# AlexanderKazakov/gcm

Hardware: AMD Instinct MI355X
Metric: Mnode-steps/sec + achieved HBM GB/s, 3D isotropic elastic 512³ CubicGrid (higher is better)
Workload: dtype f64; 1 GPU; 3-D isotropic elastic CubicGrid 512^3, borderSize 2, Courant 0.9, tau 0.9, one full time step (3 stages); global_nodes=134217728, slabs=1, launch=single process, parallelism=single, fp=fma

## Files before the change

gcm_amd/csrc/gcmx.hip:

```cpp
#include <rccl/rccl.h>

#include <algorithm>
#include <chrono>
#include <cmath>
#include <condition_variable>
#include <cstdio>
#include <cstdlib>
#include <cstring>
#include <memory>
#include <mutex>
#include <string>
#include <thread>
#include <vector>

#include "../../include/gcmx.h"
#include "common.hpp"
#include "launch.hpp"
#include "ortho.hpp"

using namespace gcmx;
static_assert(GCMX_MAX_BORDER_Q == kMaxBorderQ, "border quantity limit");
static_assert(GCMX_MAX_FACE_CONDITIONS == kMaxFaceConds && GCMX_NO_FACE_CONDITION == kNoFaceCond, "face maps");

namespace {
// ... 193 lines not shown
		if (!c->prof) return;
		b = bucket_id(c, name);
		a = take_event(c);
		e = take_event(c);
		(void)hipEventRecord(a, st);
	}
	~Timed() {
		if (b < 0) return;
		(void)hipEventRecord(e, st);
		c->pending.push_back({b, bytes, a, e});
		if (kname) c->buckets[b].kernel = kname;
	}
};

void drain_timings(gcmx_ctx* c) {
	for (auto& p : c->pending) {
		float ms = 0;
		(void)hipEventSynchronize(p.b);
		(void)hipEventElapsedTime(&ms, p.a, p.b);
		c->buckets[p.bucket].total_ms += ms;
		c->buckets[p.bucket].launches += 1;
		c->buckets[p.bucket].bytes += p.bytes;
		c->event_pool.push_back(p.a);
		c->event_pool.push_back(p.b);
	}
	c->pending.clear();
}

long long round_up(long long v, long long m) { return (v + m - 1) / m * m; }

static long long layout_pad(const char* name, long long align) {
	const char* e = std::getenv(name);
	const long long v = (e && *e) ? std::atoll(e) : 0;
	return v > 0 ? round_up(v, align) : 0;
}

long long dev_offset(const Geo& g, const int it[3]) {
	long long o = g.origin;
	for (int d = 0; d < g.D; d++) o += (long long)it[d] * g.stride[d];
	return o;
}

gcmx_status check_ctx(gcmx_ctx* c) {
	if (!c) return fail(GCMX_ERR_INVALID_ARG, "null context");
	if (hipSetDevice(c->device) != hipSuccess) return fail(GCMX_ERR_HIP, "hipSetDevice failed");
	return GCMX_OK;
}

gcmx_status build_tables(gcmx_ctx* c, double tau) {
	if (c->n_mat <= 0) return fail(GCMX_ERR_STATE, "materials not set");
	if (std::memcmp(&tau, &c->tabs_tau, sizeof(double)) == 0) return GCMX_OK;
	const int D = c->D, M = c->M, bs = c->bs;
	std::vector<AxisTable> h((size_t)c->n_mat * D);
	for (int m = 0; m < c->n_mat; m++)
		for (int s = 0; s < D; s++) {
			AxisTable& t = h[(size_t)m * D + s];
			std::memset(&t, 0, sizeof(t));
			const double* Um = &c->U[((size_t)m * D + s) * M * M];
			const double* U1m = &c->U1[((size_t)m * D + s) * M * M];
			const double* Lm = &c->L[((size_t)m * D + s) * M];
			for (int i = 0; i < M * M; i++) {
				t.U[i] = Um[i];
				t.U1[i] = U1m[i];
			}
			for (int k = 0; k < M; k++) {
				const double dx = Lm[k] * (-tau);
				const double q = std::fabs(dx) / c->desc.h[s];
// ... 2297 lines not shown
```

gcm_amd/csrc/iso.hpp:

```cpp
#pragma once

#include "common.hpp"
#include "launch.hpp"

namespace gcmx {


__host__ __device__ constexpr int sig3(int i, int j) {
	return (i <= j) ? 3 + (i * 3 - ((i - 1) * i) / 2 + j - i)
	                : 3 + (j * 3 - ((j - 1) * j) / 2 + i - j);
}
__host__ __device__ constexpr unsigned bit(int i) { return 1u << i; }

__host__ __device__ constexpr int tang1(int s) { return s == 0 ? 1 : 0; }
__host__ __device__ constexpr int tang2(int s) { return s == 2 ? 1 : 2; }
__host__ __device__ constexpr int sgn1(int s) { return s == 0 ? -1 : 1; }
__host__ __device__ constexpr int sgn2(int s) { return s == 2 ? 1 : -1; }

enum Slot : int { kZero = 0, kOne, kHalf, kA, kB, kG, kP1, kP2, kS };
struct Coef {
	int slot;
	int sign;
};
__host__ __device__ constexpr Coef cz() { return Coef{kZero, 0}; }
// ... 190 lines not shown
		for (int j = 0; j < kMaxM; j++) b[j] = sgpr_ptr(p + j * cs);
	}
	__device__ __forceinline__ void st(int j, unsigned off, double v) const {
		typedef __attribute__((address_space(1))) char* gb;
		*reinterpret_cast<gptr>(reinterpret_cast<gb>(b[j]) + (size_t)(off << 3)) = v;
	}
	__device__ __forceinline__ void st_nt(int j, unsigned off, double v) const {
		typedef __attribute__((address_space(1))) char* gb;
		__builtin_nontemporal_store(v, reinterpret_cast<gptr>(reinterpret_cast<gb>(b[j]) + (size_t)(off << 3)));
	}
};

__device__ __forceinline__ unsigned opaque_u32(unsigned x) {
	asm("" : "+v"(x));
	return x;
}
__device__ __forceinline__ double ld_b(const Planes& p, int j, unsigned boff) {
	typedef const __attribute__((address_space(1))) char* gcb;
	return *reinterpret_cast<gcptr>(reinterpret_cast<gcb>(p.b[j]) + (unsigned long long)boff);
}
__device__ __forceinline__ double ld_nt_b(const Planes& p, int j, unsigned boff) {
	typedef const __attribute__((address_space(1))) char* gcb;
	return __builtin_nontemporal_load(reinterpret_cast<gcptr>(reinterpret_cast<gcb>(p.b[j]) + (unsigned long long)boff));
}
__device__ __forceinline__ void st_b(const PlanesW& p, int j, unsigned boff, double v) {
	typedef __attribute__((address_space(1))) char* gb;
	*reinterpret_cast<gptr>(reinterpret_cast<gb>(p.b[j]) + (unsigned long long)boff) = v;
}
__device__ __forceinline__ void st_nt_b(const PlanesW& p, int j, unsigned boff, double v) {
	typedef __attribute__((address_space(1))) char* gb;
	__builtin_nontemporal_store(v, reinterpret_cast<gptr>(reinterpret_cast<gb>(p.b[j]) + (unsigned long long)boff));
}

}
```

gcm_amd/csrc/kernels_xyz.hip:

```cpp
#include "iso.hpp"

#include <cstring>
#include <string>
#include <type_traits>

namespace gcmx {
#ifndef GCMX_FMA
#define GCMX_FMA 0
#endif
#if GCMX_FMA
#define GCMX_XYZ_NS xyz_fma
#define GCMX_FP_TAG ", FMA"
#else
#define GCMX_XYZ_NS xyz_exact
#define GCMX_FP_TAG ""
#endif
namespace GCMX_XYZ_NS {


#ifndef GCMX_XYZ_MINWAVES
#define GCMX_XYZ_MINWAVES 4
#endif
#ifndef GCMX_XYZ_CHUNK
#define GCMX_XYZ_CHUNK 128
// ... 229 lines not shown
#define GCMX_TX2_BLKT 0
#endif
#if GCMX_TX2_BLKT
constexpr int kBlkMax = 8192;
__device__ unsigned long long g_tx2_blk[kBlkMax][8][2];
__device__ unsigned g_tx2_hw[kBlkMax];
#endif

#ifndef GCMX_TX2_FACEMAP
#define GCMX_TX2_FACEMAP 1
#endif
#ifndef GCMX_TX2_FACE_LDS
#define GCMX_TX2_FACE_LDS 0
#endif
#ifndef GCMX_TX2_STNT
#define GCMX_TX2_STNT 1
#endif
#ifndef GCMX_TX2_ALT
#define GCMX_TX2_ALT 1
#endif
#ifndef GCMX_TX2_NTOUTER
#define GCMX_TX2_NTOUTER 0
#endif
#ifndef GCMX_TX2_NTLOAD
#define GCMX_TX2_NTLOAD 1
#endif
#ifndef GCMX_HET_AB
#define GCMX_HET_AB 0
#endif
#ifndef GCMX_ZS_PAIRS_FIRST
#define GCMX_ZS_PAIRS_FIRST 1
#endif

#ifndef GCMX_TX2_UNROLL
#define GCMX_TX2_UNROLL 1
#endif



__host__ __device__ constexpr int wcomp(unsigned mask, int q) {
	int n = 0;
	for (int j = 0; j < 9; j++)
		if ((mask >> j) & 1u) {
			if (n == q) return j;
			n++;
		}
	return -1;
}

template <int BS, int ZT, bool KF0, bool UNI, bool FACES, bool HET, bool ZS = false>
__global__ __launch_bounds__(ZT, GCMX_TX2_MINWAVES) void k_step_tx2(
    const double* __restrict__ in, double* __restrict__ outl, Geo g, IsoAxis AX, IsoAxis AY_,
    IsoAxis AZ_, int x0, int chunk, int nplanes, int xb0, int nplanesb, FaceBC fb,
    const IsoAxis* __restrict__ mtab, const uint8_t* __restrict__ mat) {
	static_assert(!HET || (KF0 && UNI), "heterogeneous step: floor(q) = 0, Z == ZT, equal axes");
	static_assert(!ZS || (UNI && !HET), "z split: uniform medium");
	const IsoAxis& AY = UNI ? AX : AY_;
	const IsoAxis& AZ = UNI ? AX : AZ_;
	constexpr unsigned WMX = iso_window(0);
	constexpr unsigned CMX = iso_center_only(0);
	constexpr int NCX = popc9(CMX);
	constexpr unsigned WMY = iso_window(1);
	constexpr unsigned CMY = iso_center_only(1);
	constexpr int NWY = popc9(WMY);
	constexpr int NCY = popc9(CMY);
	constexpr unsigned WMZ = iso_window(2);
	constexpr int NWZ = popc9(WMZ);
	constexpr int W = 2 * BS + 1;
	constexpr int WX = W + 1;
	constexpr int LW = ZT + 2 * BS;
	static_assert(NCX >= 1 && NCY >= 1, "isotropic structure");
	constexpr bool NB = UNI && GCMX_TX2_NB;
	constexpr int NW = ZT / 64;
	constexpr int RW = 64 + 2 * BS;
	static_assert(!NB || ZT % 64 == 0, "NB needs whole waves");
	constexpr bool ZS2 = GCMX_TX2_ZS2 < 0 ? !NB : GCMX_TX2_ZS2 != 0;
	__shared__ double zl[NB ? 1 : 2][NB ? 1 : NWZ][NB ? 1 : LW];
	__shared__ double rg[NB ? NW : 1][NB ? 2 : 1][NB ? NWZ : 1][NB ? RW : 1];
	__shared__ double eg[NB ? 2 : 1][NB ? NW : 1][2][NB ? 2 : 1][NB ? NWZ : 1][BS];
	__shared__ int rdy[NB ? NW : 1];
	__shared__ double cl[BS + 1][2][NCY][ZT];
	__shared__ IsoAxis hlds[HET ? kHetMaxMaterials : 1];
	__shared__ double hode[HET ? kHetMaxMaterials : 1];
	__shared__ double flds[FACES && GCMX_TX2_FACE_LDS ? 4 : 1][9];

#if GCMX_TX2_ZPERM
	const int z = [] {
		int w = __builtin_amdgcn_readfirstlane((int)(threadIdx.x >> 6));
		if constexpr (ZT == 512) w = w < 4 ? 2 * w : 2 * (w - 4) + 1;
		return w * 64 + (int)(threadIdx.x & 63);
	}();
#else
	const int z = threadIdx.x;
#endif
#if GCMX_TX2_BLKT
	const unsigned long long blk_t0_ = __builtin_amdgcn_s_memrealtime();
#endif
	const int Y = g.sizes[1], Z = g.sizes[2];
	int x, yb, ye, xbeg, xend;
	bool rev;
	int zp = 0;
	const int nz = ZS ? g.sizes[2] / ZT : 1;
	{
		const int pa = (g.gx0 + x0) & 1, pb = (g.gx0 + xb0) & 1;
		const int npa = (nplanes + pa + 1) / 2;
		const int npair = npa + (nplanesb > 0 ? (nplanesb + pb + 1) / 2 : 0);
		const int T = (int)gridDim.x, b = (int)blockIdx.x;
		int p = xcd_order(b, T);
		if constexpr (ZS && !GCMX_ZS_PAIRS_FIRST) {
			zp = p % nz;
			p /= nz;
		}
		int q = p % npair;
		int cidx = p / npair;
		if (!ZS && chunk < 0) {
			const int co = (-chunk) & 0xFFFF, half = T >> 4;
			const int j = b >> 3, gen = j >= half ? 1 : 0;
			const int G = (b & 7) * half + (j - gen * half);
			const int ncg = (T >> 1) / npair;
			q = G % npair;
			cidx = G / npair + gen * ncg;
			const int cy = (-chunk) >> 16;
			auto start = [&](int c) { return c <= ncg ? c * co : ncg * co + (c - ncg) * cy; };
			yb = start(cidx);
			ye = min(start(cidx + 1), Y);
		}
// ... 15 lines not shown
	const bool live = UNI || z < Z;
	const int zc = live ? z : Z - 1;
	const unsigned stx = (unsigned)g.stride[0];
	const unsigned sty = (unsigned)g.stride[1];
	const long long pbase = (long long)x * g.stride[0];
	const unsigned plane = (unsigned)g.origin;
	const unsigned zo = live ? (unsigned)z : (unsigned)Z;
#if GCMX_TX2_BUF
	const Planes src(in + pbase, g.cs);
	const PlanesW out_p(outl + pbase, g.cs);
	const unsigned zpart = ZS ? (unsigned)(zp * ZT) : 0u;
	const int zg = (int)zpart + zc;
	const unsigned lv = (zpart + (unsigned)zc) * 8u, sv = (zpart + zo) * 8u;
	const unsigned pxm = plane - (unsigned)BS * stx;
	auto ldx = [&](int j, int k, int r) {
#if GCMX_TX2_PROBE_NOX
		k = k < BS ? BS : (k > BS + 1 ? BS + 1 : k);
#endif
		const int d = (k == WX - 1 && !two) ? 2 * BS : (k == 0 && !one) ? 1 : k;
		if (GCMX_TX2_NTOUTER && (k == 0 || k == WX - 1))
			return ld_nt_b(src, j, opaque_u32(lv + (pxm + (unsigned)d * stx + (unsigned)r * sty) * 8u));
		return ld_b(src, j, opaque_u32(lv + (pxm + (unsigned)d * stx + (unsigned)r * sty) * 8u));
	};
	auto ldc = [&](int j, int k, int r) {
		if constexpr (!GCMX_TX2_NTLOAD) return ldx(j, k, r);
		const int d = (k == WX - 1 && !two) ? 2 * BS : (k == 0 && !one) ? 1 : k;
		return ld_nt_b(src, j, opaque_u32(lv + (pxm + (unsigned)d * stx + (unsigned)r * sty) * 8u));
	};
	auto stz = [&](int c, int t, int y, double v) {
		const unsigned o = opaque_u32(sv + (plane + (unsigned)t * stx + (unsigned)y * sty) * 8u);
		if constexpr (GCMX_TX2_STNT) st_nt_b(out_p, c, o, v);
		else st_b(out_p, c, o, v);
	};
#else
	const unsigned base = plane + zc;
	const Planes src(in + pbase, g.cs);
	const PlanesW out_p(outl + pbase, g.cs);
	auto ldx = [&](int j, int k, int r) {
		const int d = (k == WX - 1 && !two) ? BS : (k == 0 && !one) ? 1 - BS : k - BS;
		return src.ld(j, base + (unsigned)r * sty + (unsigned)d * stx);
	};
	auto ldc = [&](int j, int k, int r) { return ldx(j, k, r); };
	auto stz = [&](int c, int t, int y, double v) { out_p.st_nt(c, plane + (unsigned)y * sty + zo + (unsigned)t * stx, v); };
#endif
	auto mt = [&](unsigned k) -> const IsoAxis& {
		if constexpr (GCMX_HET_AB >= 1) return AX;
		return hlds[k];
	};
	auto two_v = [&](int f, int j) -> double {
		if constexpr (FACES && GCMX_TX2_FACE_LDS) return flds[f][j];
		return fb.two_v[f][j];
	};
	struct GhostRule {
		unsigned mask;
		bool none;
		double two[9];
	};
	auto ghost_rule = [&](int f, int t, int pos, unsigned need) -> GhostRule {
		GhostRule r;
		r.none = false;
		if (GCMX_TX2_FACEMAP && fb.map[f]) {
			const int xx = (t == 1 && !two) ? x : (t == 0 && !one) ? x + 1 : x + t;
			const unsigned c = fb.map[f][(size_t)xx * (f < 2 ? Z : Y) + pos];
			r.none = c == kNoFaceCond;
			const FaceCond& fc = fb.conds[r.none ? 0u : c];
			r.mask = r.none ? 0u : fc.mask;
#pragma unroll
			for (int j = 0; j < 9; j++)
				if ((need >> j) & 1u) r.two[j] = r.none ? 0.0 : fc.two_v[j];
		} else {
			r.mask = fb.mask[f];
#pragma unroll
			for (int j = 0; j < 9; j++)
				if ((need >> j) & 1u) r.two[j] = two_v(f, j);
		}
		return r;
	};
	auto ghost = [](const GhostRule& r, int j, double v) -> double {
		return r.none ? 0.0 : ((r.mask >> j) & 1u) ? -v + r.two[j] : v;
	};

	const int wv = z >> 6, ln = z & 63;
	const bool seam_own = ZS && ((zp > 0 && z < BS) || (zp < nz - 1 && z >= ZT - BS));
	if constexpr (NB) {
		if (ln < BS || ln >= 64 - BS) {
			const int hs = ln < BS ? ln : ln + 2 * BS;
#pragma unroll
			for (int t = 0; t < 2; t++)
#pragma unroll
				for (int q = 0; q < NWZ; q++) rg[wv][t][q][hs] = 0.0;
		}
		if (z < NW) rdy[z] = -1;
		__syncthreads();
	} else if (z < 2 * BS) {
		const int gslot = (z < BS) ? z : (Z + z);
#pragma unroll
		for (int t = 0; t < 2; t++)
#pragma unroll
			for (int q = 0; q < NWZ; q++) zl[t][q][gslot] = 0.0;
	}

	typedef double PairWin[2][WX];
	auto pair_load = [&](auto PC, PairWin& w, int r) {
		constexpr int P = decltype(PC)::value;
#pragma unroll
		for (int k = 0; k < WX; k++) {
			w[0][k] = ldx(pair_vel(0, P), k, r);
			w[1][k] = ldx(pair_sig(0, P), k, r);
		}
	};
	auto pair_rows = [&](auto PC, const PairWin& w, double (&rr)[2][9], const IsoAxis& A0, const IsoAxis& A1,
	                     bool same) {
		constexpr int P = decltype(PC)::value;
		if (KF0 && !same) {
#pragma unroll
			for (int t = 0; t < 2; t++)
				pair_update<0, BS, true, P>(
				    t ? A1 : A0, [&](int j, int o) { return j == pair_vel(0, P) ? w[0][t + BS + o] : w[1][t + BS + o]; },
				    rr[t][2 * P], rr[t][2 * P + 1]);
		} else if constexpr (KF0 && !GCMX_LAGRANGE) {
			const IsoAxis& AS = A0;
			const double* c = (P == 0) ? AS.c1 : AS.c2;
			double im[2][2], ip[2][2];
#pragma unroll
			for (int v = 0; v < 2; v++) {
				double D[BS + 1][WX];
#pragma unroll
				for (int k = 0; k < WX; k++) D[0][k] = w[v][k];
#pragma unroll
				for (int i = 1; i <= BS; i++)
#pragma unroll
					for (int k = 0; k + i < WX; k++) D[i][k] = (D[i - 1][k + 1] - D[i - 1][k]) * c[i - 1];
#pragma unroll
				for (int t = 0; t < 2; t++) {
					const int m = t + BS;
					double a = D[0][m], b = D[0][m];
#pragma unroll
					for (int i = 1; i <= BS; i++) {
						a += D[i][m];
						b = (i % 2) ? b - D[i][m - i] : b + D[i][m - i];
					}
					ip[v][t] = vlimit(a, D[0][m], D[0][m + 1]);
					im[v][t] = vlimit(b, D[0][m], D[0][m - 1]);
				}
			}
#pragma unroll
			for (int t = 0; t < 2; t++) {
				rr[t][2 * P] = RowSum<0, false, 2 * P>::go(
				    AS, [&](int j) { return j == pair_vel(0, P) ? im[0][t] : im[1][t]; }, 0.0, true);
				rr[t][2 * P + 1] = RowSum<0, false, 2 * P + 1>::go(
				    AS, [&](int j) { return j == pair_vel(0, P) ? ip[0][t] : ip[1][t]; }, 0.0, true);
			}
		} else {
#pragma unroll
			for (int t = 0; t < 2; t++)
				pair_update<0, BS, KF0, P>(
				    t ? A1 : A0, [&](int j, int o) { return j == pair_vel(0, P) ? w[0][t + BS + o] : w[1][t + BS + o]; },
				    rr[t][2 * P], rr[t][2 * P + 1]);
		}
	};
	auto sched_fence = [] { __builtin_amdgcn_sched_barrier(0); };
	using P0 = std::integral_constant<int, 0>;
	using P1 = std::integral_constant<int, 1>;
	using P2 = std::integral_constant<int, 2>;
	struct XPre {
		PairWin a, b;
	};
	auto cv_load = [&](double (&cv)[2][9], int r) {
#pragma unroll
		for (int t = 0; t < 2; t++)
#pragma unroll
			for (int j = 0; j < 9; j++)
				if ((CMX >> j) & 1u) cv[t][j] = ldc(j, BS + t, r);
	};
	auto x_load_ahead = [&](XPre& pre, int r) {
		pair_load(P0{}, pre.a, r);
		pair_load(P1{}, pre.b, r);
	};
	auto mat_of = [&](int t, int r) -> unsigned {
		const int xx = (t == 1 && !two) ? x : (t == 0 && !one) ? x + 1 : x + t;
		const int rr_ = r < 0 ? 0 : (r < Y ? r : Y - 1);
		return mat[((size_t)xx * Y + rr_) * Z + z];
	};
	auto x_compute = [&](const XPre& pre, const PairWin& wc, const double (&cv)[2][9], double (&xr)[2][9],
	                     const IsoAxis& A0, const IsoAxis& A1, bool same) {
		double rr[2][9], n0[2][9];
		pair_rows(P0{}, pre.a, rr, A0, A1, same);
		pair_rows(P1{}, pre.b, rr, A0, A1, same);
		sched_fence();
		pair_rows(P2{}, wc, rr, A0, A1, same);
#pragma unroll
		for (int t = 0; t < 2; t++) {
			n0[t][pair_vel(0, 0)] = pre.a[0][t + BS];
			n0[t][pair_sig(0, 0)] = pre.a[1][t + BS];
			n0[t][pair_vel(0, 1)] = pre.b[0][t + BS];
			n0[t][pair_sig(0, 1)] = pre.b[1][t + BS];
			n0[t][pair_vel(0, 2)] = wc[0][t + BS];
			n0[t][pair_sig(0, 2)] = wc[1][t + BS];
		}
		sched_fence();
#pragma unroll
		for (int t = 0; t < 2; t++) {
			const IsoAxis& A = t ? A1 : A0;
			center_update<0>(A, [&](int j) { return ((WMX >> j) & 1u) ? n0[t][j] : cv[t][j]; }, rr[t]);
			u1_apply<0>(A, rr[t], xr[t]);
		}
	};
	auto key_of = [&](int r) -> unsigned {
		if constexpr (GCMX_HET_AB >= 2) return 0u;
		return mat_of(0, r) | (mat_of(1, r) << 8);
	};
	auto x_stage = [&](const XPre& pre, int r, double (&xr)[2][9], unsigned key) {
		PairWin wc;
		double cv[2][9];
		TX2_PRIO_HI();
		pair_load(P2{}, wc, r);
		cv_load(cv, r);
		TX2_PRIO_LO();
		sched_fence();
		if constexpr (HET) {
			const unsigned m0 = key & 255u, m1 = key >> 8;
			x_compute(pre, wc, cv, xr, mt(m0), mt(m1), m0 == m1);
		} else {
			x_compute(pre, wc, cv, xr, AX, AX, true);
		}
	};

	double win[2][NWY][W];
	unsigned hk[W];
#pragma unroll
	for (int k = 0; k < W; k++) hk[k] = 0;
	if constexpr (HET) {
		for (int i = z; i < kHetMaxMaterials * (int)(sizeof(IsoAxis) / 4); i += ZT)
			reinterpret_cast<unsigned*>(hlds)[i] = reinterpret_cast<const unsigned*>(mtab)[i];
		if (fb.ode_on && fb.ode_f && z < kHetMaxMaterials) hode[z] = fb.ode_f[z];
	}
	if constexpr (FACES && GCMX_TX2_FACE_LDS) {
#pragma unroll
		for (int c = 0; c < 36; c++)
			if (z == c) flds[c / 9][c % 9] = fb.two_v[c / 9][c % 9];
	}
	if constexpr (HET || (FACES && GCMX_TX2_FACE_LDS)) __syncthreads();
	auto run = [&](auto RV) {
	constexpr bool REV = decltype(RV)::value;
	constexpr int S = REV ? -1 : 1;
	auto cl_at = [&](int r) { return &cl[(r + 2 * BS + 2) % (BS + 1)][0][0][z]; };
	auto push = [&](const double (&xr)[2][9], int slot, int r) {
		double* cp = cl_at(r);
#pragma unroll
		for (int t = 0; t < 2; t++)
#pragma unroll
			for (int j = 0; j < 9; j++) {
				if ((WMY >> j) & 1u) win[t][wslot(WMY, j)][slot] = xr[t][j];
				if ((CMY >> j) & 1u) cp[(t * NCY + wslot(CMY, j)) * ZT] = xr[t][j];
			}
	};
	auto mirror_slot = [&](int k, int ks, int f) {
#pragma unroll
		for (int t = 0; t < 2; t++) {
			const GhostRule gr = ghost_rule(f, t, zg, WMY);
#pragma unroll
			for (int q = 0; q < NWY; q++) {
				double v = 0.0;
#pragma unroll
				for (int kk = 0; kk < W; kk++)
					if (kk == ks) v = win[t][q][kk];
				const double gv = ghost(gr, wcomp(WMY, q), v);
#pragma unroll
				for (int kk = 0; kk < W; kk++)
					if (kk == k) win[t][q][kk] = gv;
			}
		}
	};
	const int y0 = REV ? ye - 1 : yb;
#pragma unroll
	for (int k = 0; k < W; k++) {
		const int r = y0 + S * (k - BS);
		double xr[2][9];
		if (r >= 0 && r < Y) {
// ... 42 lines not shown
			else go(AY);
		}
	};
	auto z_ghosts = [&](int y, const double (&yv)[2][9], auto&& put) {
		const int wu = __builtin_amdgcn_readfirstlane(z >> 6);
#pragma unroll
		for (int side = 0; side < 2; side++) {
			const int Zl = ZS ? ZT : Z;
			if (ZS && (side ? zp != nz - 1 : zp != 0)) continue;
			const int lo = side ? Zl - 1 - BS : 1, hi = side ? Zl - 2 : BS;
			if (!((fb.on >> (2 + side)) & 1u) || wu * 64 > hi || wu * 64 + 63 < lo) continue;
			if (z < lo || z > hi) continue;
#pragma unroll
			for (int t = 0; t < 2; t++) {
				const GhostRule gr = ghost_rule(2 + side, t, y, WMZ);
#pragma unroll
				for (int j = 0; j < 9; j++)
					if ((WMZ >> j) & 1u) put(side, t, wslot(WMZ, j), ghost(gr, j, yv[t][j]));
			}
		}
	};
	auto publish = [&](int it, int y, const double (&yv)[2][9]) {
		const int es = it & 1;
		if constexpr (NB) {
			double* egp = ln < BS ? &eg[es][wv][0][0][0][ln] : &eg[es][wv][1][0][0][ln - (64 - BS)];
			const bool edge = ln < BS || ln >= 64 - BS;
			asm volatile("" ::: "memory");
#pragma unroll
			for (int t = 0; t < 2; t++)
#pragma unroll
				for (int j = 0; j < 9; j++)
					if ((WMZ >> j) & 1u) {
						const int q = wslot(WMZ, j);
						rg[wv][t][q][BS + ln] = yv[t][j];
						if (edge) egp[(t * NWZ + q) * BS] = yv[t][j];
					}
			if constexpr (FACES)
				z_ghosts(y, yv, [&](int side, int t, int q, double v) {
					if (side == 0) rg[0][t][q][BS - z] = v;
					else rg[NW - 1][t][q][BS + 2 * ((ZS ? ZT : Z) - 1) - z - 64 * (NW - 1)] = v;
				});
			asm volatile("s_waitcnt lgkmcnt(0)" ::: "memory");
			__hip_atomic_store(&rdy[wv], it, __ATOMIC_RELAXED, __HIP_MEMORY_SCOPE_WORKGROUP);
		} else {
			__syncthreads();
#pragma unroll
			for (int t = 0; t < 2; t++)
#pragma unroll
				for (int j = 0; j < 9; j++)
					if ((WMZ >> j) & 1u) {
						const int q = wslot(WMZ, j);
						if constexpr (FACES) {
							if (UNI || z < Z || z >= Z + BS) zl[t][q][BS + z] = live ? yv[t][j] : 0.0;
						} else {
							zl[t][q][BS + z] = live ? yv[t][j] : 0.0;
						}
					}
			if constexpr (FACES)
				z_ghosts(y, yv, [&](int side, int t, int q, double v) {
					if (side == 0) zl[t][q][BS - z] = v;
					else zl[t][q][BS + 2 * (Z - 1) - z] = v;
				});
			__syncthreads();
		}
	};
	auto collect = [&](int it) {
		if constexpr (NB && NW > 1) {
			const int es = it & 1;
			for (;;) {
				const int a = wv > 0 ? __hip_atomic_load(&rdy[wv - 1], __ATOMIC_RELAXED, __HIP_MEMORY_SCOPE_WORKGROUP) : it;
				const int b =
				    wv < NW - 1 ? __hip_atomic_load(&rdy[wv + 1], __ATOMIC_RELAXED, __HIP_MEMORY_SCOPE_WORKGROUP) : it;
				if (__builtin_amdgcn_readfirstlane(min(a, b)) >= it) break;
				if constexpr (GCMX_TX2_SLEEP > 0) __builtin_amdgcn_s_sleep(GCMX_TX2_SLEEP);
			}
			asm volatile("" ::: "memory");
			if (ln < BS && wv > 0) {
#pragma unroll
				for (int t = 0; t < 2; t++)
#pragma unroll
					for (int q = 0; q < NWZ; q++) rg[wv][t][q][ln] = eg[es][wv - 1][1][t][q][ln];
			}
			if (ln >= 64 - BS && wv < NW - 1) {
#pragma unroll
				for (int t = 0; t < 2; t++)
#pragma unroll
					for (int q = 0; q < NWZ; q++) rg[wv][t][q][ln + 2 * BS] = eg[es][wv + 1][0][t][q][ln - (64 - BS)];
			}
			asm volatile("" ::: "memory");
		}
	};
	auto z_stage_store = [&](int t, int y, const double (&yv)[2][9]) {
		double zv[9];
		auto go = [&](const IsoAxis& A) {
			if constexpr (NB)
				node_update<2, BS, KF0>(
				    A, [&](int j, int o) { return rg[wv][t][wslot(WMZ, j)][BS + ln + o]; },
				    [&](int j) { return ((WMZ >> j) & 1u) ? rg[wv][t][wslot(WMZ, j)][BS + ln] : yv[t][j]; }, zv);
			else
				node_update<2, BS, KF0>(
				    A, [&](int j, int o) { return zl[t][wslot(WMZ, j)][BS + z + o]; },
				    [&](int j) { return ((WMZ >> j) & 1u) ? zl[t][wslot(WMZ, j)][BS + z] : yv[t][j]; }, zv);
		};
		if constexpr (HET) go(mt(t ? hk[BS] >> 8 : hk[BS] & 255u));
		else go(AZ);
		if (fb.ode_on) {
			double f = fb.ode;
			if constexpr (HET)
				if (fb.ode_f) f = hode[t ? hk[BS] >> 8 : hk[BS] & 255u];
#pragma unroll
			for (int c = 3; c < 9; c++) zv[c] = zv[c] * f;
		}
		if ((t == 0 ? one : two) && !(ZS && seam_own)) {
#pragma unroll
			for (int c = 0; c < 9; c++) stz(c, t, y, live ? zv[c] : 0.0);
		}
	};
	auto x_enter = [&](int y, const XPre& pre, unsigned kn) {
#pragma unroll
		for (int t = 0; t < 2; t++)
#pragma unroll
			for (int q = 0; q < NWY; q++)
#pragma unroll
				for (int o = 0; o < W - 1; o++) win[t][q][o] = win[t][q][o + 1];
		if constexpr (HET) {
#pragma unroll
			for (int o = 0; o < W - 1; o++) hk[o] = hk[o + 1];
			hk[W - 1] = kn;
		}
		double xr[2][9];
		sched_fence();
		const int r = y + S * (BS + 1);
		x_stage(pre, clamp_row(r), xr, kn);
		push(xr, W - 1, r);
		sched_fence();
		if constexpr (FACES) {
			const int f = r < 0 ? 0 : 1;
			if ((r < 0 || r >= Y) && ((fb.on >> f) & 1u)) {
				const int ks = BS + S * ((r < 0 ? -r : 2 * (Y - 1) - r) - (y + S));
				if (ks >= 0 && ks < W) mirror_slot(W - 1, ks, f);
			}
		}
	};
	auto row = [&](int y, int it) {
		double yv[2][9];
		XPre pre;
		const int rn = clamp_row(y + S * (BS + 1));
		unsigned kn = 0;
		if constexpr (HET) kn = key_of(rn);
		y_stage(y, yv);
		TX2_T(0);
		publish(it, y, yv);
		TX2_T(2);
		if constexpr (ZS2) {
			sched_fence();
			pair_load(P0{}, pre.a, rn);
			sched_fence();
		} else {
			sched_fence();
			TX2_PRIO_HI();
			x_load_ahead(pre, rn);
			TX2_PRIO_LO();
			sched_fence();
		}
		TX2_T(6);
		collect(it);
		TX2_T(4);
#pragma unroll
		for (int t = 0; t < 2; t++) {
			if constexpr (ZS2) {
				if (t == 1) {
					sched_fence();
					pair_load(P1{}, pre.b, rn);
					sched_fence();
				}
			}
			z_stage_store(t, y, yv);
		}
		TX2_T(3);
		x_enter(y, pre, kn);
		TX2_T(5);
	};
#if GCMX_TX2_UNROLL > 1
#pragma unroll GCMX_TX2_UNROLL
#endif
	for (int it = 0; it < ye - yb; it++) row(REV ? ye - 1 - it : yb + it, it);
#if GCMX_TX2_BLKT
	if ((threadIdx.x & 63) == 0 && blockIdx.x < (unsigned)kBlkMax && threadIdx.x < 512) {
		const unsigned long long t1 = __builtin_amdgcn_s_memrealtime();
		g_tx2_blk[blockIdx.x][threadIdx.x / 64][0] = blk_t0_;
		g_tx2_blk[blockIdx.x][threadIdx.x / 64][1] = t1;
		if (threadIdx.x == 0) g_tx2_hw[blockIdx.x] = __builtin_amdgcn_s_getreg((31 << 11) | 4);
	}
#endif
#if GCMX_TX2_DIAG
	if ((threadIdx.x & 63) == 0) {
		const int wv = threadIdx.x / 64;
		for (int i = 0; i < 8; i++) atomicAdd(&g_tx2_diag[wv][i], dt_[i]);
	}
#endif
	};
	if (rev) run(std::true_type{});
	else run(std::false_type{});
}

template <int BS, bool KF0, bool FACES>
__global__ __launch_bounds__(256) void k_zseam(const double* __restrict__ in, double* __restrict__ outl, Geo g,
                                                IsoAxis A, int x0, int nplanes, int xb0, int nplanesb, int zt,
                                                int chunk, FaceBC fb) {
	const unsigned ode_on = fb.ode_on;
	const double ode = fb.ode;
// ... 81 lines not shown
				for (int k = 3; k < 9; k++) zv[k] = zv[k] * ode;
			}
			const long long off = base + (long long)y * sty;
#pragma unroll
			for (int k = 0; k < 9; k++) __builtin_nontemporal_store(zv[k], outl + k * cs + off);
		}
#pragma unroll
		for (int j = 0; j < 9; j++)
#pragma unroll
			for (int k = 0; k < W - 1; k++) win[j][k] = win[j][k + 1];
		double xr[9];
		const int r = y + BS + 1;
		if (r < Y) xstage(r, xr);
		else
#pragma unroll
			for (int j = 0; j < 9; j++) xr[j] = 0.0;
#pragma unroll
		for (int j = 0; j < 9; j++) win[j][W - 1] = xr[j];
		if constexpr (FACES) {
			if (r >= Y && ((fb.on >> 1) & 1u)) {
				const int ks = BS + (2 * (Y - 1) - r) - (y + 1);
				if (ks >= 0 && ks < W) mirror(W - 1, ks, 1);
			}
		}
	}
}


static bool same_axis(const IsoAxis& p, const IsoAxis& q) {
	static_assert(sizeof(IsoAxis) == 18 * 8 + 2 * 4, "IsoAxis has padding");
	return std::memcmp(&p, &q, sizeof(IsoAxis)) == 0;
}

template <int BS, int ZT, bool KF0, bool UNI, bool FACES, bool HET, bool ZS = false>
static const char* tx2_name() {
	static const std::string s = "k_step_tx2<" + std::to_string(BS) + ", " + std::to_string(ZT) + ", " +
	                             (KF0 ? "KF0" : "!KF0") + ", " + (UNI ? "UNI" : "!UNI") + ", " +
	                             (FACES ? "FACES" : "!FACES") + (HET ? ", HET" : "") + (ZS ? ", ZS" : "") +
	                             GCMX_FP_TAG + ">";
	return s.c_str();
}
template <int BS, int ZT, bool KF0, bool UNI>
static const char* xyz_name() {
	static const std::string s = "k_fused_xyz<" + std::to_string(BS) + ", " + std::to_string(ZT) + ", " +
	                             (KF0 ? "KF0" : "!KF0") + ", " + (UNI ? "UNI" : "!UNI") + GCMX_FP_TAG + ">";
	return s.c_str();
}

static int tx2_chunk_for(int Y, int npair, int req, int slots) {
	if (req > 0) return Y <= req ? Y : req;
	for (int t = 1024; t >= 16; t /= 2) {
		const int ch = Y < t ? Y : t;
		if (10LL * npair * ((Y + ch - 1) / ch) >= 9LL * slots) return ch;
	}
	return Y < 16 ? Y : 16;
}

static int device_cus();
static int tx2_gen2(int Y, int npair, int chunk, int T, int per_cu) {
	static const int pct = [] {
		const char* e = std::getenv("GCMX_TX2_GEN2");
		return e ? std::atoi(e) : GCMX_TX2_GEN2_DEFAULT;
	}();
	if (pct <= 50 || pct >= 100 || per_cu != 2 || T != 2 * device_cus() || T % 16 || (T / 2) % npair) return chunk;
	const int nchunk = T / npair;
	if (Y % chunk || Y / chunk != nchunk) return chunk;
	const int ncg = nchunk / 2, two = Y / ncg;
	if (two * ncg != Y) return chunk;
	const int co = (two * pct + 50) / 100, cy = two - co;
	if (cy < 2 * 2 + 1 || co > 0xFFFF) return chunk;
	return -(co | (cy << 16));
}

static int device_cus() {
	static int n = [] {
		int dev = 0, v = 0;
		if (hipGetDevice(&dev) != hipSuccess ||
		    hipDeviceGetAttribute(&v, hipDeviceAttributeMultiprocessorCount, dev) != hipSuccess || v <= 0)
			v = 256;
		return v;
	}();
	return n;
}

static int xyz_chunk_for(int Y, int nplanes, int req, int start = GCMX_XYZ_CHUNK, int min_blocks = 1024) {
	int chunk = req > 0 ? req : start;
	if (req <= 0)
		while (chunk > 16 && (long long)((Y + chunk - 1) / chunk) * nplanes < min_blocks) chunk /= 2;
	return Y <= chunk ? Y : chunk;
}

template <int BS, int P, bool FACES>
static void launch_zs(const double* in, double* out, const Geo& g, const IsoAxis* a, int x0, int x1, int xb0, int xb1,
                      hipStream_t st, int req_chunk, const FaceBC* fb, const char** kname) {
	const int nz = g.sizes[2] / P, nb = xb1 > xb0 ? xb1 - xb0 : 0;
	const int npair = (x1 - x0 + ((g.gx0 + x0) & 1) + 1) / 2 + (nb > 0 ? (nb + ((g.gx0 + xb0) & 1) + 1) / 2 : 0);
	const int chunk = req_chunk > 0 ? std::min(req_chunk, g.sizes[1]) : std::min(128, g.sizes[1]);
	const dim3 grid(((g.sizes[1] + chunk - 1) / chunk) * npair * nz);
	const FaceBC none{};
	const FaceBC& f = fb ? *fb : none;
	hipLaunchKernelGGL((k_step_tx2<BS, P, true, true, FACES, false, true>), grid, dim3(P), 0, st, in, out, g, a[0],
	                   a[1], a[2], x0, chunk, x1 - x0, xb0, nb, f, nullptr, nullptr);
	const int np = (x1 - x0) + nb, pb = 256 / (4 * BS), sch = std::min(64, g.sizes[1]);
	const long long nblk = (long long)((np + pb - 1) / pb) * (nz - 1) * ((g.sizes[1] + sch - 1) / sch);
	hipLaunchKernelGGL((k_zseam<BS, true, FACES>), dim3((unsigned)nblk), dim3(256), 0, st, in, out, g, a[0], x0,
	                   x1 - x0, xb0, nb, P, sch, f);
	*kname = tx2_name<BS, P, true, true, FACES, false, true>();
}

template <int BS, int ZT>
static void launch_xyz_t(const double* in, double* out, const Geo& g, const IsoAxis* a, int x0,
                         int x1, int xb0, int xb1, hipStream_t st, int req_chunk, const FaceBC* fb,
                         const char** kname, const HetMaterials* het) {
	bool kf0 = true;
	for (int s = 0; s < 3; s++) kf0 = kf0 && a[s].kf1 == 0 && a[s].kf2 == 0;
	const bool uni = kf0 && g.sizes[2] == ZT && same_axis(a[0], a[1]) && same_axis(a[0], a[2]);
	if constexpr (BS <= 2 && ZT <= 512) {
		if (GCMX_XYZ_TX2 || fb) {
			const int nb = xb1 > xb0 ? xb1 - xb0 : 0;
			const int npair = (x1 - x0 + ((g.gx0 + x0) & 1) + 1) / 2 +
			                  (nb > 0 ? (nb + ((g.gx0 + xb0) & 1) + 1) / 2 : 0);
			const int chunk = tx2_chunk_for(g.sizes[1], npair, req_chunk, device_cus() * (512 / ZT));
			const dim3 grid(((g.sizes[1] + chunk - 1) / chunk) * npair);
			const int cparam = req_chunk > 0 ? chunk : tx2_gen2(g.sizes[1], npair, chunk, (int)grid.x, 512 / ZT);
			const FaceBC none{};
			const FaceBC& f = fb ? *fb : none;
			const IsoAxis* mt = het ? het->tab : nullptr;
			const uint8_t* mi = het ? het->ids : nullptr;
			auto go = [&](auto K, const char* name) {
				hipLaunchKernelGGL(K, grid, dim3(ZT), 0, st, in, out, g, a[0], a[1], a[2], x0, cparam, x1 - x0, xb0,
				                   nb, f, mt, mi);
				*kname = name;
			};
			if (het) {
				if (fb && fb->on) go(k_step_tx2<BS, ZT, true, true, true, true>, tx2_name<BS, ZT, true, true, true, true>());
				else go(k_step_tx2<BS, ZT, true, true, false, true>, tx2_name<BS, ZT, true, true, false, true>());
				return;
			}
			if (fb && fb->on) {
				if (uni) go(k_step_tx2<BS, ZT, true, true, true, false>, tx2_name<BS, ZT, true, true, true, false>());
				else if (kf0) go(k_step_tx2<BS, ZT, true, false, true, false>, tx2_name<BS, ZT, true, false, true, false>());
				else go(k_step_tx2<BS, ZT, false, false, true, false>, tx2_name<BS, ZT, false, false, true, false>());
			} else {
				if (uni) go(k_step_tx2<BS, ZT, true, true, false, false>, tx2_name<BS, ZT, true, true, false, false>());
				else if (kf0) go(k_step_tx2<BS, ZT, true, false, false, false>, tx2_name<BS, ZT, true, false, false, false>());
				else go(k_step_tx2<BS, ZT, false, false, false, false>, tx2_name<BS, ZT, false, false, false, false>());
			}
			return;
		}
	}
	if (xb1 > xb0) {
		launch_xyz_t<BS, ZT>(in, out, g, a, x0, x1, 0, 0, st, req_chunk, fb, kname, het);
		x0 = xb0;
		x1 = xb1;
	}
	const int chunk = xyz_chunk_for(g.sizes[1], x1 - x0, req_chunk);
	const dim3 grid(((g.sizes[1] + chunk - 1) / chunk) * (x1 - x0));
	if (uni) {
		hipLaunchKernelGGL((k_fused_xyz<BS, ZT, true, true>), grid, dim3(ZT), 0, st, in, out, g, a[0], a[1],
		                   a[2], x0, chunk, x1 - x0);
		*kname = xyz_name<BS, ZT, true, true>();
	} else if (kf0) {
		hipLaunchKernelGGL((k_fused_xyz<BS, ZT, true, false>), grid, dim3(ZT), 0, st, in, out, g, a[0], a[1],
		                   a[2], x0, chunk, x1 - x0);
		*kname = xyz_name<BS, ZT, true, false>();
	} else {
		hipLaunchKernelGGL((k_fused_xyz<BS, ZT, false, false>), grid, dim3(ZT), 0, st, in, out, g, a[0], a[1],
		                   a[2], x0, chunk, x1 - x0);
		*kname = xyz_name<BS, ZT, false, false>();
	}
}

template <int BS>
static bool launch_xyz_bs(const double* in, double* out, const Geo& g, const IsoAxis* a, int x0,
                          int x1, int xb0, int xb1, hipStream_t st, int ch, const FaceBC* fb,
                          const char** kn, const HetMaterials* het) {
	const int Z = g.sizes[2];
// ... 111 lines not shown
```

gcm_amd/csrc/launch.hpp:

```cpp
#pragma once

#include "common.hpp"

#include <string>

namespace gcmx {

void set_last_error(const std::string& msg);

bool launch_stage_generic(const double* cur, double* nxt, const Geo& g, int s,
                          const AxisTable* tabs, const uint8_t* mat, hipStream_t st);
void launch_fill_random(double* cur, const Geo& g, const int gstart[3], long long GY,
                        long long GZ, uint64_t seed, hipStream_t st);
void launch_copy_box(double* dst, const Geo& gd, const double* src, const Geo& gs,
                     const int dmin[3], const int smin[3], const int ext[3], hipStream_t st);
void launch_scale_stress(double* cur, const Geo& g, const uint8_t* mat_d, const double* f_d,
                         double f0, hipStream_t st);
struct OdeFactors {
	int n;
	double f[255];
};
void launch_set_factors(double* dst_d, const OdeFactors& v, hipStream_t st);
constexpr int kMaxBorderQ = 16;
struct BorderQ {
// ... 12 lines not shown
struct IsoAxis {
	double a, b, g;
	double p1, p2, s;
	double c1[3], c2[3];
	double w1[3], w2[3];
	int kf1, kf2;
};
inline void lagrange_weights(const double* c, int bs, double* w) {
	w[0] = w[1] = w[2] = 0.0;
	if (bs == 1) {
		w[0] = 1.0 - c[0];
		w[1] = c[0];
	} else if (bs == 2) {
		const double c01 = c[0] * c[1];
		w[0] = (1.0 - c[0]) + c01;
		w[1] = c[0] - 2.0 * c01;
		w[2] = c01;
	}
}
bool iso_axis_extract(int s, const double* U, const double* U1, const double* L, IsoAxis& A);
constexpr int kStep2dMaxBs = 5;
bool iso2_axis_extract(int s, const double* U, const double* U1, const double* L, IsoAxis& A);
bool step2d_supported(const Geo& g);
bool step2d_iso_supported(const Geo& g);
struct Face2 {
	unsigned on;
	unsigned mask[2];
	double two_v[2][5];
};
bool launch_step2d(const double* cur, double* nxt, const Geo& g, const AxisTable* tabs, const IsoAxis* iso,
                   hipStream_t st, const char** kname, const Face2* faces = nullptr);
bool fast_layout_ok(const Geo& g);
bool onepass_layout_ok(const Geo& g);
bool launch_march(const double* cur, double* nxt, const Geo& g, int s, const IsoAxis& A,
                  int x0, int x1, hipStream_t st);
bool launch_line_z(const double* cur, double* nxt, const Geo& g, const IsoAxis& A, int x0,
                   int x1, hipStream_t st);
bool fused_supported(const Geo& g);
struct FaceCond {
	unsigned mask;
	unsigned pad_;
	double two_v[9];
};
constexpr int kHetMaxMaterials = 32;
constexpr int kMaxFaceConds = 8;
constexpr uint8_t kNoFaceCond = 255;
struct FaceBC {
	unsigned on;
	unsigned mask[4];
	double two_v[4][9];
	unsigned ode_on;
	double ode;
	const double* ode_f;
	const uint8_t* map[4];
	const FaceCond* conds;
};
struct FaceTables {
	int n;
	BorderQ bq[kMaxFaceConds];
	FaceCond fc[kMaxFaceConds];
};
void launch_set_face_tables(BorderQ* bq_d, FaceCond* fc_d, const FaceTables& t, hipStream_t st);
bool fused_faces_supported(const Geo& g);
struct HetMaterials {
	const IsoAxis* tab;
	const uint8_t* ids;
// ... 20 lines not shown
```

Before: 37160 Mnode-steps/s.

## Use 16-byte paired loads/stores in tx2 step kernel with lane-pair permutation

Adds a wide variant of the tx2 step kernel where each lane handles two adjacent z nodes, doing 128-bit dpair global loads and stores. permlane32_swap exchanges the halves back to the per-node arrangement, and the LDS row indexing is remapped to an interleaved layout. The aim is fewer memory instructions and better HBM transaction efficiency, at the cost of extra permute instructions, register pressure and more complex seam handling. It is only enabled when the layout is even-aligned and the pointers are 16-byte aligned.

```diff
diff --git a/gcm_amd/csrc/gcmx.hip b/gcm_amd/csrc/gcmx.hip
--- a/gcm_amd/csrc/gcmx.hip
+++ b/gcm_amd/csrc/gcmx.hip
@@ -249,7 +249,7 @@
 static long long layout_pad(const char* name, long long align) {
 	const char* e = std::getenv(name);
 	const long long v = (e && *e) ? std::atoll(e) : 0;
-	return v > 0 ? round_up(v, align) : 0;
+	return v <= 0 ? 0 : (v & 1) ? v : round_up(v, align);
 }
 
 long long dev_offset(const Geo& g, const int it[3]) {
diff --git a/gcm_amd/csrc/iso.hpp b/gcm_amd/csrc/iso.hpp
--- a/gcm_amd/csrc/iso.hpp
+++ b/gcm_amd/csrc/iso.hpp
@@ -246,4 +246,34 @@
 	__builtin_nontemporal_store(v, reinterpret_cast<gptr>(reinterpret_cast<gb>(p.b[j]) + (unsigned long long)boff));
 }
 
-}
+typedef double dpair __attribute__((ext_vector_type(2)));
+__device__ __forceinline__ dpair ld2_b(const Planes& p, int j, unsigned boff) {
+	typedef const __attribute__((address_space(1))) char* gcb;
+	typedef const __attribute__((address_space(1))) dpair* gcp2;
+	return *reinterpret_cast<gcp2>(reinterpret_cast<gcb>(p.b[j]) + (unsigned long long)boff);
+}
+__device__ __forceinline__ dpair ld2_nt_b(const Planes& p, int j, unsigned boff) {
+	typedef const __attribute__((address_space(1))) char* gcb;
+	typedef const __attribute__((address_space(1))) dpair* gcp2;
+	return __builtin_nontemporal_load(reinterpret_cast<gcp2>(reinterpret_cast<gcb>(p.b[j]) + (unsigned long long)boff));
+}
+__device__ __forceinline__ void st2_b(const PlanesW& p, int j, unsigned boff, dpair v) {
+	typedef __attribute__((address_space(1))) char* gb;
+	typedef __attribute__((address_space(1))) dpair* gp2;
+	*reinterpret_cast<gp2>(reinterpret_cast<gb>(p.b[j]) + (unsigned long long)boff) = v;
+}
+__device__ __forceinline__ void st2_nt_b(const PlanesW& p, int j, unsigned boff, dpair v) {
+	typedef __attribute__((address_space(1))) char* gb;
+	typedef __attribute__((address_space(1))) dpair* gp2;
+	__builtin_nontemporal_store(v, reinterpret_cast<gp2>(reinterpret_cast<gb>(p.b[j]) + (unsigned long long)boff));
+}
+__device__ __forceinline__ void half_swap(double& a, double& b) {
+	typedef unsigned u32x2 __attribute__((ext_vector_type(2)));
+	const u32x2 x = __builtin_bit_cast(u32x2, a), y = __builtin_bit_cast(u32x2, b);
+	const u32x2 lo = __builtin_amdgcn_permlane32_swap(x.x, y.x, false, false);
+	const u32x2 hi = __builtin_amdgcn_permlane32_swap(x.y, y.y, false, false);
+	a = __builtin_bit_cast(double, u32x2{lo.x, hi.x});
+	b = __builtin_bit_cast(double, u32x2{lo.y, hi.y});
+}
+
+}
diff --git a/gcm_amd/csrc/kernels_xyz.hip b/gcm_amd/csrc/kernels_xyz.hip
--- a/gcm_amd/csrc/kernels_xyz.hip
+++ b/gcm_amd/csrc/kernels_xyz.hip
@@ -285,6 +285,9 @@
 #define GCMX_ZS_PAIRS_FIRST 1
 #endif
 
+#ifndef GCMX_TX2_WIDE
+#define GCMX_TX2_WIDE 1
+#endif
 #ifndef GCMX_TX2_UNROLL
 #define GCMX_TX2_UNROLL 1
 #endif
@@ -301,7 +304,7 @@
 	return -1;
 }
 
-template <int BS, int ZT, bool KF0, bool UNI, bool FACES, bool HET, bool ZS = false>
+template <int BS, int ZT, bool KF0, bool UNI, bool FACES, bool HET, bool ZS = false, bool WD = false>
 __global__ __launch_bounds__(ZT, GCMX_TX2_MINWAVES) void k_step_tx2(
     const double* __restrict__ in, double* __restrict__ outl, Geo g, IsoAxis AX, IsoAxis AY_,
     IsoAxis AZ_, int x0, int chunk, int nplanes, int xb0, int nplanesb, FaceBC fb,
@@ -325,8 +328,10 @@
 	static_assert(NCX >= 1 && NCY >= 1, "isotropic structure");
 	constexpr bool NB = UNI && GCMX_TX2_NB;
 	constexpr int NW = ZT / 64;
-	constexpr int RW = 64 + 2 * BS;
 	static_assert(!NB || ZT % 64 == 0, "NB needs whole waves");
+	constexpr bool WIDE = WD && NB && GCMX_TX2_WIDE && GCMX_TX2_BUF;
+	static_assert(!WD || WIDE, "wide instance launched without its path compiled in");
+	constexpr int RW = WIDE ? 68 : 64 + 2 * BS;
 	constexpr bool ZS2 = GCMX_TX2_ZS2 < 0 ? !NB : GCMX_TX2_ZS2 != 0;
 	__shared__ double zl[NB ? 1 : 2][NB ? 1 : NWZ][NB ? 1 : LW];
 	__shared__ double rg[NB ? NW : 1][NB ? 2 : 1][NB ? NWZ : 1][NB ? RW : 1];
@@ -341,10 +346,11 @@
 	const int z = [] {
 		int w = __builtin_amdgcn_readfirstlane((int)(threadIdx.x >> 6));
 		if constexpr (ZT == 512) w = w < 4 ? 2 * w : 2 * (w - 4) + 1;
-		return w * 64 + (int)(threadIdx.x & 63);
+		const int l = (int)(threadIdx.x & 63);
+		return w * 64 + (WIDE ? ((l & 31) << 1) | (l >> 5) : l);
 	}();
 #else
-	const int z = threadIdx.x;
+	const int z = WIDE ? (int)((threadIdx.x & ~63u) | ((threadIdx.x & 31u) << 1) | ((threadIdx.x >> 5) & 1u)) : (int)threadIdx.x;
 #endif
 #if GCMX_TX2_BLKT
 	const unsigned long long blk_t0_ = __builtin_amdgcn_s_memrealtime();
@@ -426,6 +432,20 @@
 		if constexpr (GCMX_TX2_STNT) st_nt_b(out_p, c, o, v);
 		else st_b(out_p, c, o, v);
 	};
+	const bool hsel = (threadIdx.x & 32u) != 0;
+	const unsigned lw = (zpart + (unsigned)(z & ~63) + 2u * (threadIdx.x & 31u)) * 8u;
+	auto ldw = [&](int j, int ka, int kb, int r, bool nt) {
+		auto cl_ = [&](int k) { return (k == WX - 1 && !two) ? 2 * BS : (k == 0 && !one) ? 1 : k; };
+		const unsigned pa = (pxm + (unsigned)cl_(ka) * stx) * 8u, pb = (pxm + (unsigned)cl_(kb) * stx) * 8u;
+		const unsigned o = opaque_u32(lw + (hsel ? pb : pa) + (unsigned)r * sty * 8u);
+		return nt ? ld2_nt_b(src, j, o) : ld2_b(src, j, o);
+	};
+	auto stw = [&](int c, int y, double v0, double v1) {
+		const unsigned o = opaque_u32(lw + (plane + (hsel ? stx : 0u) + (unsigned)y * sty) * 8u);
+		const dpair v = {v0, v1};
+		if constexpr (GCMX_TX2_STNT) st2_nt_b(out_p, c, o, v);
+		else st2_b(out_p, c, o, v);
+	};
 #else
 	const unsigned base = plane + zc;
 	const Planes src(in + pbase, g.cs);
@@ -476,9 +496,18 @@
 
 	const int wv = z >> 6, ln = z & 63;
 	const bool seam_own = ZS && ((zp > 0 && z < BS) || (zp < nz - 1 && z >= ZT - BS));
+	auto rs = [](int c) { return WIDE ? (c >> 1) + ((c & 1) ? 35 : 1) : BS + c; };
+	const int rs0 = rs(ln), rs1 = rs(ln + 1);
+	auto rso = [&](int o) { return !WIDE ? rs0 + o : (o & 1) ? rs1 + ((o - 1) >> 1) : rs0 + (o >> 1); };
+	const bool seam_pair = [&] {
+		const int cb = (z & ~63) + 2 * (int)(threadIdx.x & 31u);
+		auto sc = [&](int c) { return (zp > 0 && c < BS) || (zp < nz - 1 && c >= ZT - BS); };
+		return ZS && sc(cb) && sc(cb + 1);
+	}();
+	const int ci = WIDE ? (int)threadIdx.x : z;
 	if constexpr (NB) {
 		if (ln < BS || ln >= 64 - BS) {
-			const int hs = ln < BS ? ln : ln + 2 * BS;
+			const int hs = rs(ln < BS ? ln - BS : ln + BS);
 #pragma unroll
 			for (int t = 0; t < 2; t++)
 #pragma unroll
@@ -497,10 +526,33 @@
 	typedef double PairWin[2][WX];
 	auto pair_load = [&](auto PC, PairWin& w, int r) {
 		constexpr int P = decltype(PC)::value;
+		if constexpr (WIDE) {
+#if GCMX_TX2_BUF
+#pragma unroll
+			for (int m = 0; m < WX / 2; m++) {
+				const dpair a = ldw(pair_vel(0, P), 2 * m, 2 * m + 1, r, false);
+				const dpair b = ldw(pair_sig(0, P), 2 * m, 2 * m + 1, r, false);
+				w[0][2 * m] = a.x, w[0][2 * m + 1] = a.y;
+				w[1][2 * m] = b.x, w[1][2 * m + 1] = b.y;
+			}
+#endif
+			return;
+		}
 #pragma unroll
 		for (int k = 0; k < WX; k++) {
 			w[0][k] = ldx(pair_vel(0, P), k, r);
 			w[1][k] = ldx(pair_sig(0, P), k, r);
+		}
+	};
+	auto pair_fix = [&](const PairWin& w, PairWin& u) {
+#pragma unroll
+		for (int v = 0; v < 2; v++) {
+#pragma unroll
+			for (int k = 0; k < WX; k++) u[v][k] = w[v][k];
+			if constexpr (WIDE) {
+#pragma unroll
+				for (int m = 0; m < WX / 2; m++) half_swap(u[v][2 * m], u[v][2 * m + 1]);
+			}
 		}
 	};
 	auto pair_rows = [&](auto PC, const PairWin& w, double (&rr)[2][9], const IsoAxis& A0, const IsoAxis& A1,
@@ -561,6 +613,17 @@
 		PairWin a, b;
 	};
 	auto cv_load = [&](double (&cv)[2][9], int r) {
+		if constexpr (WIDE) {
+#if GCMX_TX2_BUF
+#pragma unroll
+			for (int j = 0; j < 9; j++)
+				if ((CMX >> j) & 1u) {
+					const dpair v = ldw(j, BS, BS + 1, r, GCMX_TX2_NTLOAD != 0);
+					cv[0][j] = v.x, cv[1][j] = v.y;
+				}
+#endif
+			return;
+		}
 #pragma unroll
 		for (int t = 0; t < 2; t++)
 #pragma unroll
@@ -576,23 +639,33 @@
 		const int rr_ = r < 0 ? 0 : (r < Y ? r : Y - 1);
 		return mat[((size_t)xx * Y + rr_) * Z + z];
 	};
-	auto x_compute = [&](const XPre& pre, const PairWin& wc, const double (&cv)[2][9], double (&xr)[2][9],
+	auto x_compute = [&](const XPre& pre, const PairWin& wc_, const double (&cv_)[2][9], double (&xr)[2][9],
 	                     const IsoAxis& A0, const IsoAxis& A1, bool same) {
-		double rr[2][9], n0[2][9];
-		pair_rows(P0{}, pre.a, rr, A0, A1, same);
-		pair_rows(P1{}, pre.b, rr, A0, A1, same);
+		double rr[2][9], n0[2][9], cv[2][9];
+		PairWin pa, pb, wc;
+		pair_fix(pre.a, pa);
+		pair_rows(P0{}, pa, rr, A0, A1, same);
+		pair_fix(pre.b, pb);
+		pair_rows(P1{}, pb, rr, A0, A1, same);
 		sched_fence();
+		pair_fix(wc_, wc);
 		pair_rows(P2{}, wc, rr, A0, A1, same);
 #pragma unroll
 		for (int t = 0; t < 2; t++) {
-			n0[t][pair_vel(0, 0)] = pre.a[0][t + BS];
-			n0[t][pair_sig(0, 0)] = pre.a[1][t + BS];
-			n0[t][pair_vel(0, 1)] = pre.b[0][t + BS];
-			n0[t][pair_sig(0, 1)] = pre.b[1][t + BS];
+			n0[t][pair_vel(0, 0)] = pa[0][t + BS];
+			n0[t][pair_sig(0, 0)] = pa[1][t + BS];
+			n0[t][pair_vel(0, 1)] = pb[0][t + BS];
+			n0[t][pair_sig(0, 1)] = pb[1][t + BS];
 			n0[t][pair_vel(0, 2)] = wc[0][t + BS];
 			n0[t][pair_sig(0, 2)] = wc[1][t + BS];
 		}
 		sched_fence();
+#pragma unroll
+		for (int j = 0; j < 9; j++)
+			if ((CMX >> j) & 1u) {
+				cv[0][j] = cv_[0][j], cv[1][j] = cv_[1][j];
+				if constexpr (WIDE) half_swap(cv[0][j], cv[1][j]);
+			}
 #pragma unroll
 		for (int t = 0; t < 2; t++) {
 			const IsoAxis& A = t ? A1 : A0;
@@ -638,7 +711,7 @@
 	auto run = [&](auto RV) {
 	constexpr bool REV = decltype(RV)::value;
 	constexpr int S = REV ? -1 : 1;
-	auto cl_at = [&](int r) { return &cl[(r + 2 * BS + 2) % (BS + 1)][0][0][z]; };
+	auto cl_at = [&](int r) { return &cl[(r + 2 * BS + 2) % (BS + 1)][0][0][ci]; };
 	auto push = [&](const double (&xr)[2][9], int slot, int r) {
 		double* cp = cl_at(r);
 #pragma unroll
@@ -747,13 +820,13 @@
 				for (int j = 0; j < 9; j++)
 					if ((WMZ >> j) & 1u) {
 						const int q = wslot(WMZ, j);
-						rg[wv][t][q][BS + ln] = yv[t][j];
+						rg[wv][t][q][rs0] = yv[t][j];
 						if (edge) egp[(t * NWZ + q) * BS] = yv[t][j];
 					}
 			if constexpr (FACES)
 				z_ghosts(y, yv, [&](int side, int t, int q, double v) {
-					if (side == 0) rg[0][t][q][BS - z] = v;
-					else rg[NW - 1][t][q][BS + 2 * ((ZS ? ZT : Z) - 1) - z - 64 * (NW - 1)] = v;
+					if (side == 0) rg[0][t][q][rs(-z)] = v;
+					else rg[NW - 1][t][q][rs(2 * ((ZS ? ZT : Z) - 1) - z - 64 * (NW - 1))] = v;
 				});
 			asm volatile("s_waitcnt lgkmcnt(0)" ::: "memory");
 			__hip_atomic_store(&rdy[wv], it, __ATOMIC_RELAXED, __HIP_MEMORY_SCOPE_WORKGROUP);
@@ -794,24 +867,23 @@
 #pragma unroll
 				for (int t = 0; t < 2; t++)
 #pragma unroll
-					for (int q = 0; q < NWZ; q++) rg[wv][t][q][ln] = eg[es][wv - 1][1][t][q][ln];
+					for (int q = 0; q < NWZ; q++) rg[wv][t][q][rs(ln - BS)] = eg[es][wv - 1][1][t][q][ln];
 			}
 			if (ln >= 64 - BS && wv < NW - 1) {
 #pragma unroll
 				for (int t = 0; t < 2; t++)
 #pragma unroll
-					for (int q = 0; q < NWZ; q++) rg[wv][t][q][ln + 2 * BS] = eg[es][wv + 1][0][t][q][ln - (64 - BS)];
+					for (int q = 0; q < NWZ; q++) rg[wv][t][q][rs(ln + BS)] = eg[es][wv + 1][0][t][q][ln - (64 - BS)];
 			}
 			asm volatile("" ::: "memory");
 		}
 	};
-	auto z_stage_store = [&](int t, int y, const double (&yv)[2][9]) {
-		double zv[9];
+	auto z_stage_store = [&](int t, int y, const double (&yv)[2][9], double (&zv)[9]) {
 		auto go = [&](const IsoAxis& A) {
 			if constexpr (NB)
 				node_update<2, BS, KF0>(
-				    A, [&](int j, int o) { return rg[wv][t][wslot(WMZ, j)][BS + ln + o]; },
-				    [&](int j) { return ((WMZ >> j) & 1u) ? rg[wv][t][wslot(WMZ, j)][BS + ln] : yv[t][j]; }, zv);
+				    A, [&](int j, int o) { return rg[wv][t][wslot(WMZ, j)][rso(o)]; },
+				    [&](int j) { return ((WMZ >> j) & 1u) ? rg[wv][t][wslot(WMZ, j)][rs0] : yv[t][j]; }, zv);
 			else
 				node_update<2, BS, KF0>(
 				    A, [&](int j, int o) { return zl[t][wslot(WMZ, j)][BS + z + o]; },
@@ -826,10 +898,21 @@
 #pragma unroll
 			for (int c = 3; c < 9; c++) zv[c] = zv[c] * f;
 		}
+		if constexpr (WIDE) return;
 		if ((t == 0 ? one : two) && !(ZS && seam_own)) {
 #pragma unroll
 			for (int c = 0; c < 9; c++) stz(c, t, y, live ? zv[c] : 0.0);
 		}
+	};
+	auto z_store_wide = [&](int y, double (&zv)[2][9]) {
+#if GCMX_TX2_BUF
+#pragma unroll
+		for (int c = 0; c < 9; c++) half_swap(zv[0][c], zv[1][c]);
+		if ((hsel ? two : one) && !seam_pair) {
+#pragma unroll
+			for (int c = 0; c < 9; c++) stw(c, y, zv[0][c], zv[1][c]);
+		}
+#endif
 	};
 	auto x_enter = [&](int y, const XPre& pre, unsigned kn) {
 #pragma unroll
@@ -858,7 +941,7 @@
 		}
 	};
 	auto row = [&](int y, int it) {
-		double yv[2][9];
+		double yv[2][9], zv[2][9];
 		XPre pre;
 		const int rn = clamp_row(y + S * (BS + 1));
 		unsigned kn = 0;
@@ -890,8 +973,9 @@
 					sched_fence();
 				}
 			}
-			z_stage_store(t, y, yv);
-		}
+			z_stage_store(t, y, yv, zv[t]);
+		}
+		if constexpr (WIDE) z_store_wide(y, zv);
 		TX2_T(3);
 		x_enter(y, pre, kn);
 		TX2_T(5);
@@ -1039,13 +1123,17 @@
 	return std::memcmp(&p, &q, sizeof(IsoAxis)) == 0;
 }
 
-template <int BS, int ZT, bool KF0, bool UNI, bool FACES, bool HET, bool ZS = false>
+template <int BS, int ZT, bool KF0, bool UNI, bool FACES, bool HET, bool ZS = false, bool WD = false>
 static const char* tx2_name() {
 	static const std::string s = "k_step_tx2<" + std::to_string(BS) + ", " + std::to_string(ZT) + ", " +
 	                             (KF0 ? "KF0" : "!KF0") + ", " + (UNI ? "UNI" : "!UNI") + ", " +
 	                             (FACES ? "FACES" : "!FACES") + (HET ? ", HET" : "") + (ZS ? ", ZS" : "") +
-	                             GCMX_FP_TAG + ">";
+	                             (UNI && !WD ? ", N8" : "") + GCMX_FP_TAG + ">";
 	return s.c_str();
+}
+constexpr bool kTx2Wide = (GCMX_TX2_WIDE != 0) & (GCMX_TX2_NB != 0) & (GCMX_TX2_BUF != 0);
+static bool tx2_wide_ok(const Geo& g, const double* in, const double* out) {
+	return kTx2Wide && wide_layout_ok(g) && (((uintptr_t)in | (uintptr_t)out) & 15u) == 0;
 }
 template <int BS, int ZT, bool KF0, bool UNI>
 static const char* xyz_name() {
@@ -1106,13 +1194,18 @@
 	const dim3 grid(((g.sizes[1] + chunk - 1) / chunk) * npair * nz);
 	const FaceBC none{};
 	const FaceBC& f = fb ? *fb : none;
-	hipLaunchKernelGGL((k_step_tx2<BS, P, true, true, FACES, false, true>), grid, dim3(P), 0, st, in, out, g, a[0],
-	                   a[1], a[2], x0, chunk, x1 - x0, xb0, nb, f, nullptr, nullptr);
+	auto go = [&](auto WDC) {
+		constexpr bool WD = decltype(WDC)::value;
+		hipLaunchKernelGGL((k_step_tx2<BS, P, true, true, FACES, false, true, WD>), grid, dim3(P), 0, st, in, out, g,
+		                   a[0], a[1], a[2], x0, chunk, x1 - x0, xb0, nb, f, nullptr, nullptr);
+		*kname = tx2_name<BS, P, true, true, FACES, false, true, WD>();
+	};
+	if (tx2_wide_ok(g, in, out)) go(std::integral_constant<bool, kTx2Wide>{});
+	else go(std::false_type{});
 	const int np = (x1 - x0) + nb, pb = 256 / (4 * BS), sch = std::min(64, g.sizes[1]);
 	const long long nblk = (long long)((np + pb - 1) / pb) * (nz - 1) * ((g.sizes[1] + sch - 1) / sch);
 	hipLaunchKernelGGL((k_zseam<BS, true, FACES>), dim3((unsigned)nblk), dim3(256), 0, st, in, out, g, a[0], x0,
 	                   x1 - x0, xb0, nb, P, sch, f);
-	*kname = tx2_name<BS, P, true, true, FACES, false, true>();
 }
 
 template <int BS, int ZT>
@@ -1139,17 +1232,25 @@
 				                   nb, f, mt, mi);
 				*kname = name;
 			};
+			const bool wide = tx2_wide_ok(g, in, out);
+			auto go_uni = [&](auto FC, auto HC) {
+				constexpr bool F = decltype(FC)::value, H = decltype(HC)::value;
+				constexpr bool W = kTx2Wide && !(H && BS == 2) && ZT != 256;
+				if (wide && W) go(k_step_tx2<BS, ZT, true, true, F, H, false, W>,
+				                  tx2_name<BS, ZT, true, true, F, H, false, W>());
+				else go(k_step_tx2<BS, ZT, true, true, F, H>, tx2_name<BS, ZT, true, true, F, H>());
+			};
 			if (het) {
-				if (fb && fb->on) go(k_step_tx2<BS, ZT, true, true, true, true>, tx2_name<BS, ZT, true, true, true, true>());
-				else go(k_step_tx2<BS, ZT, true, true, false, true>, tx2_name<BS, ZT, true, true, false, true>());
+				if (fb && fb->on) go_uni(std::true_type{}, std::true_type{});
+				else go_uni(std::false_type{}, std::true_type{});
 				return;
 			}
 			if (fb && fb->on) {
-				if (uni) go(k_step_tx2<BS, ZT, true, true, true, false>, tx2_name<BS, ZT, true, true, true, false>());
+				if (uni) go_uni(std::true_type{}, std::false_type{});
 				else if (kf0) go(k_step_tx2<BS, ZT, true, false, true, false>, tx2_name<BS, ZT, true, false, true, false>());
 				else go(k_step_tx2<BS, ZT, false, false, true, false>, tx2_name<BS, ZT, false, false, true, false>());
 			} else {
-				if (uni) go(k_step_tx2<BS, ZT, true, true, false, false>, tx2_name<BS, ZT, true, true, false, false>());
+				if (uni) go_uni(std::false_type{}, std::false_type{});
 				else if (kf0) go(k_step_tx2<BS, ZT, true, false, false, false>, tx2_name<BS, ZT, true, false, false, false>());
 				else go(k_step_tx2<BS, ZT, false, false, false, false>, tx2_name<BS, ZT, false, false, false, false>());
 			}
diff --git a/gcm_amd/csrc/launch.hpp b/gcm_amd/csrc/launch.hpp
--- a/gcm_amd/csrc/launch.hpp
+++ b/gcm_amd/csrc/launch.hpp
@@ -68,6 +68,9 @@
                    hipStream_t st, const char** kname, const Face2* faces = nullptr);
 bool fast_layout_ok(const Geo& g);
 bool onepass_layout_ok(const Geo& g);
+inline bool wide_layout_ok(const Geo& g) {
+	return g.D == 3 && ((g.origin | g.stride[0] | g.stride[1] | g.cs) & 1) == 0;
+}
 bool launch_march(const double* cur, double* nxt, const Geo& g, int s, const IsoAxis& A,
                   int x0, int x1, hipStream_t st);
 bool launch_line_z(const double* cur, double* nxt, const Geo& g, const IsoAxis& A, int x0,
```

Result: faster. 38120 Mnode-steps/s, median of 6 (+2.6%).
